# ViskaWei/VIT

Measured on AMD Instinct MI355X. Metric: images/sec ViT-B/16 224^2 bf16 train step, higher is better.
Workload: dtype bf16

## Files before the change

### include/vit_amd.h

```cpp
#ifndef VIT_AMD_H_
#define VIT_AMD_H_

#include <stddef.h>
#include <stdint.h>

#ifdef __cplusplus
extern "C" {
#endif

#define VIT_AMD_VERSION 100

typedef struct vit_ctx* vit_handle;
typedef void* vit_stream;

typedef enum { VIT_OK = 0, VIT_ERR_ARG = -1, VIT_ERR_HIP = -2, VIT_ERR_UNSUPPORTED = -3, VIT_ERR_WORKSPACE = -4 } vit_status;
typedef enum { VIT_F32 = 0, VIT_BF16 = 1 } vit_dtype;
typedef enum { VIT_ACT_NONE = 0, VIT_ACT_GELU = 1, VIT_ACT_DGELU = 2, VIT_ACT_GELU_GRAD = 3, VIT_ACT_MUL_AUX = 4 } vit_act;
typedef enum { VIT_LOSS_MSE = 0, VIT_LOSS_L1 = 1, VIT_LOSS_CE = 2, VIT_LOSS_SOFT_CE = 3, VIT_LOSS_BCE = 4 } vit_loss;

int vit_version(void);
const char* vit_last_error(void);

int vit_create(vit_handle* out, int device);
int vit_destroy(vit_handle h);
// ... 107 lines not shown
int vit_grad_sqnorm_acc(vit_handle h, const float* g, int64_t n, float* out, vit_stream stream);
int vit_adamw_step(vit_handle h, float* p, const float* g, float* m, float* v, void* p_bf16, int64_t n, float lr,
                   float beta1, float beta2, float eps, float weight_decay, int step, const float* sqnorm,
                   float max_norm, vit_stream stream);

#ifdef __cplusplus
}
#endif

#include "vit_amd_cov.h"
#include "vit_amd_optim.h"
#include "vit_amd_ema.h"
#include "vit_amd_droppath.h"
#include "vit_amd_layerscale.h"
#include "vit_amd_mix.h"

#endif
```

### vit_amd/_cabi.py

```python
from __future__ import annotations

import ctypes as C
import os
import re
import threading

_HERE = os.path.dirname(os.path.abspath(__file__))
LIB_PATH = os.environ.get("VIT_AMD_LIB") or os.path.join(_HERE, "lib", "libvit_amd.so")
HEADER_PATH = os.path.join(os.path.dirname(_HERE), "include", "vit_amd.h")

VIT_OK, VIT_ERR_WORKSPACE = 0, -4
VIT_F32, VIT_BF16 = 0, 1
ACT_NONE, ACT_GELU, ACT_DGELU, ACT_GELU_GRAD, ACT_MUL_AUX = 0, 1, 2, 3, 4
LOSS_MSE, LOSS_L1, LOSS_CE = 0, 1, 2
LOSS_SOFT_CE, LOSS_BCE = 3, 4
MIX_LABELS_F32, MIX_LABELS_I64 = 0, 1


class VitError(RuntimeError):
    pass


class GemmDesc(C.Structure):
    _fields_ = [
# ... 38 lines not shown

_P, _I, _F, _U64, _I64, _SZ = C.c_void_p, C.c_int, C.c_float, C.c_uint64, C.c_int64, C.c_size_t

_PROTOS = {
    "vit_version": [],
    "vit_last_error": [],
    "vit_create": [C.POINTER(_P), _I],
    "vit_destroy": [_P],
    "vit_set_workspace": [_P, _P, _SZ],
    "vit_workspace_needed": [],
    "vit_set_option": [C.c_char_p, _I],
    "vit_handle_set_option": [_P, C.c_char_p, _I],
    "vit_step_state_bind": [_P, _P],
    "vit_step_advance": [_P, _U64, _F, _F, _P],
    "vit_gemm": [_P, C.POINTER(GemmDesc), _P],
    "vit_last_gemm_kernel": [],
    "vit_linear_fwd": [_P, _P, _P, _P, _P, _I, _I, _I, _I, _I, _P, _F, _U64, _U64, _P, _P],
    "vit_linear_bwd_dx": [_P, _P, _P, _P, _I, _I, _I, _I, _P, _P],
    "vit_linear_bwd_dw": [_P, _P, _P, _P, _I, _I, _I, _I, _P],
    "vit_layernorm_fwd": [_P, _P, _P, _P, _P, _I, _P, _P, _I, _I, _F, _P],
    "vit_layernorm_fwd_residual": [_P, _P, _P, _I, _P, _P, _P, _P, _I, _P, _P, _I, _I, _F, _P],
    "vit_linear_bwd_dw_rows": [_P, _P, _I64, _P, _I64, _I, _P, _I, _I, _I, _I64, _I64, _P],
    "vit_colsum_rows": [_P, _P, _I, _I64, _P, _I, _I, _I64, _I64, _P],
    "vit_layernorm_fwd_residual_rows": [_P, _P, _I64, _P, _I, _P, _P, _P, _P, _I, _P, _P, _I, _I, _F, _P],
    "vit_layernorm_bwd_rows": [_P, _P, _I, _P, _P, _P, _P, _P, _I64, _P, _P, _P, _I, _I, _P, _I, _P, _F, _U64, _U64, _I64, _P],
    "vit_layernorm_bwd": [_P, _P, _I, _P, _P, _P, _P, _P, _P, _P, _P, _I, _I, _P],
    "vit_layernorm_bwd_fused": [_P, _P, _I, _P, _P, _P, _P, _P, _P, _P, _P, _I, _I, _P, _I, _P, _F, _U64, _U64, _P],
    "vit_attention_fwd": [_P, _P, _P, _P, _P, _I, _I, _I, _I, _I, _F, _F, _U64, _U64, _P],
    "vit_attention_bwd": [_P, _P, _P, _P, _P, _P, _P, _P, _I, _I, _I, _I, _I, _F, _F, _U64, _U64, _P, _P],
    "vit_attention_probs": [_P, _P, _P, _I, _I, _I, _I, _I, _F, _P],
# ... 156 lines not shown
```

### vit_amd/build.py

```python
from __future__ import annotations

import hashlib
import os
import subprocess
import sys
from concurrent.futures import ThreadPoolExecutor

HERE = os.path.dirname(os.path.abspath(__file__))
ROOT = os.path.dirname(HERE)
CSRC = os.path.join(HERE, "csrc")
OBJ = os.path.join(CSRC, "_build")
LIBDIR = os.path.join(HERE, "lib")
LIB = os.path.join(LIBDIR, "libvit_amd.so")
ARCH = "gfx950"
SOURCES = ["api.hip", "gemm.hip", "gemm2.hip", "layernorm.hip", "attention.hip", "attention_tiled.hip", "attention_resident.hip",
           "attention_pipe.hip", "attention_f32.hip", "elementwise.hip", "covariance.hip", "optim.hip", "ema.hip", "layerscale.hip", "mix.hip"]
HEADERS = [os.path.join(CSRC, "common.h"), os.path.join(CSRC, "attention.h"), os.path.join(ROOT, "include", "vit_amd.h"),
           os.path.join(ROOT, "include", "vit_amd_cov.h"), os.path.join(ROOT, "include", "vit_amd_optim.h"),
           os.path.join(ROOT, "include", "vit_amd_ema.h"), os.path.join(ROOT, "include", "vit_amd_droppath.h"),
           os.path.join(ROOT, "include", "vit_amd_layerscale.h"), os.path.join(ROOT, "include", "vit_amd_mix.h")]


def _hipcc() -> str:
    for c in (os.environ.get("HIPCC"), "/opt/rocm/bin/hipcc", "hipcc"):
        if c and (os.path.isabs(c) and os.path.exists(c) or not os.path.isabs(c)):
            return c
    raise RuntimeError("hipcc not found")


def _stamp(paths) -> str:
    h = hashlib.sha256()
    for p in paths:
        with open(p, "rb") as f:
            h.update(f.read())
    return h.hexdigest()
# ... 49 lines not shown
```

### vit_amd/csrc/api.hip

```cpp
#include <stdarg.h>
#include <stdio.h>
#include <string.h>

#include <algorithm>

#include "common.h"

struct vit_ctx {
  int device;
  void* ws;
  size_t ws_bytes;
  const void* step_state;
  int num_cus;
  int reserve_cus;
  int grad_accumulate;
  int lamb_passes;
};

namespace vit {

extern int g_gemm2_mode;
extern int g_attn_split, g_attn_bwd_fused;

static thread_local char g_err[512] = "";
thread_local char g_last_gemm[96] = "";

void set_error(const char* fmt, ...) {
  va_list ap;
  va_start(ap, fmt);
  vsnprintf(g_err, sizeof(g_err), fmt, ap);
  va_end(ap);
// ... 5 lines not shown
int ctx_num_cus(vit_handle h) {
  static int dflt = 0;
  if (h) return std::max(1, h->num_cus - (h->reserve_cus >= 0 ? h->reserve_cus : g_reserve_cus));
  if (!dflt) {
    int dev = 0, n = 0;
    if (hipGetDevice(&dev) == hipSuccess && hipDeviceGetAttribute(&n, hipDeviceAttributeMultiprocessorCount, dev) == hipSuccess && n > 0)
      dflt = n;
    else
      dflt = 256;
  }
  return std::max(1, dflt - g_reserve_cus);
}

int ctx_grad_accumulate(vit_handle h) { return h ? h->grad_accumulate : 0; }
int ctx_lamb_passes(vit_handle h) { return h ? h->lamb_passes : 7; }

static thread_local size_t g_ws_needed = 0;
void* ctx_claim(vit_handle h, size_t need_bytes, const char* who) {
  const size_t have = h ? h->ws_bytes : 0;
  if (h && h->ws && have >= need_bytes) return h->ws;
  g_ws_needed = need_bytes;
  set_error("%s: needs %zu workspace bytes, have %zu", who, need_bytes, have);
  return nullptr;
}

}

extern "C" {

int vit_version(void) { return VIT_AMD_VERSION; }
// ... 8 lines not shown
  VIT_HIP(hipGetDeviceCount(&n));
  VIT_CHECK(device >= 0 && device < n, VIT_ERR_ARG, "vit_create: device %d out of range (%d visible)", device, n);
  hipDeviceProp_t prop;
  VIT_HIP(hipGetDeviceProperties(&prop, device));
  VIT_CHECK(strncmp(prop.gcnArchName, "gfx950", 6) == 0, VIT_ERR_UNSUPPORTED,
            "vit_create: device %d is %s; this library is built for gfx950 (MI355X) only", device, prop.gcnArchName);
  vit_ctx* c = new vit_ctx();
  c->device = device;
  c->ws = nullptr;
  c->ws_bytes = 0;
  c->step_state = nullptr;
  c->num_cus = prop.multiProcessorCount > 0 ? prop.multiProcessorCount : 256;
  c->reserve_cus = -1;
  c->grad_accumulate = 0;
  c->lamb_passes = 7;
  *out = c;
  return VIT_OK;
}

int vit_destroy(vit_handle h) {
  delete h;
  return VIT_OK;
}

const char* vit_last_gemm_kernel(void) { return vit::g_last_gemm; }

int vit_set_option(const char* name, int value) {
  VIT_CHECK(name, VIT_ERR_ARG, "vit_set_option: null name");
  if (strcmp(name, "gemm_core") == 0) {
    VIT_CHECK(value == 0 || value == 1 || value == 5, VIT_ERR_ARG,
// ... 28 lines not shown
  if (strcmp(name, "reserve_cus") == 0) {
    VIT_CHECK(value >= -1 && value <= 128, VIT_ERR_ARG, "vit_handle_set_option: reserve_cus takes -1 (process default) or 0 .. 128");
    h->reserve_cus = value;
    return VIT_OK;
  }
  if (strcmp(name, "grad_accumulate") == 0) {
    VIT_CHECK(value == 0 || value == 1, VIT_ERR_ARG, "vit_handle_set_option: grad_accumulate takes 0 or 1");
    h->grad_accumulate = value;
    return VIT_OK;
  }
  if (strcmp(name, "lamb_passes") == 0) {
    VIT_CHECK(value >= 1 && value <= 7, VIT_ERR_ARG, "vit_handle_set_option: lamb_passes takes 1 .. 7 (bits: moments 1, ratios 2, apply 4)");
    h->lamb_passes = value;
    return VIT_OK;
  }
  vit::set_error("vit_handle_set_option: '%s' is not a per-handle option (reserve_cus, grad_accumulate, lamb_passes)", name);
  return VIT_ERR_ARG;
}

int vit_step_state_bind(vit_handle h, void* state) {
  VIT_CHECK(h, VIT_ERR_ARG, "vit_step_state_bind: null handle");
  VIT_CHECK(((uintptr_t)state & 15) == 0, VIT_ERR_ARG, "vit_step_state_bind: state must be 16-byte aligned");
  h->step_state = state;
  return VIT_OK;
}

int vit_set_workspace(vit_handle h, void* ws, size_t bytes) {
  VIT_CHECK(h, VIT_ERR_ARG, "vit_set_workspace: null handle");
  VIT_CHECK(((uintptr_t)ws & 255) == 0, VIT_ERR_ARG, "vit_set_workspace: workspace must be 256-byte aligned");
  h->ws = ws;
  h->ws_bytes = bytes;
// ... 5 lines not shown
```

### vit_amd/csrc/common.h

```cpp
#pragma once
#include <hip/hip_runtime.h>
#include <stdint.h>

#include "../../include/vit_amd.h"

namespace vit {

typedef __attribute__((ext_vector_type(8))) short bf16x8;
typedef __attribute__((ext_vector_type(4))) short bf16x4;
typedef __attribute__((ext_vector_type(4))) float f32x4;
typedef __attribute__((ext_vector_type(4))) int i32x4;
typedef __attribute__((ext_vector_type(2))) int i32x2;
typedef __attribute__((ext_vector_type(4))) unsigned u32x4;
typedef __attribute__((ext_vector_type(2))) unsigned u32x2;

#define LDS_AS __attribute__((address_space(3)))

void set_error(const char* fmt, ...);
extern thread_local char g_last_gemm[96];
#define VIT_CHECK(cond, code, ...)            \
  do {                                         \
    if (!(cond)) {                             \
      ::vit::set_error(__VA_ARGS__);           \
      return (code);                           \
// ... 256 lines not shown
  int accumulate;
  int grad_accumulate;
  int scratch;
  DropCfg drop;
  int drs;
  KRows kr;
  size_t slab_bytes, colsum_bytes, scratch_off, need;
  char* ws;
  char symbol[96];
};
int gemm_plan(vit_handle h, const vit_gemm_desc* d, KRows kr, GemmPlan* pl);
bool pp_plan(vit_handle h, const vit_gemm_desc* d, GemmPlan* pl);
int pp_launch(const GemmPlan& pl, const vit_gemm_desc* d, hipStream_t st);
int gemm_launch(vit_handle h, const vit_gemm_desc* d, hipStream_t st, int k_row_stride = 0, int k_rows = 0);

template <class Args>
static inline void fill_gemm_args(Args& a, const GemmPlan& pl, const vit_gemm_desc* d) {
  a.A = (const char*)d->A; a.B = (const char*)d->B; a.C = (char*)d->C;
  a.lda = d->lda; a.ldb = d->ldb; a.ldc = d->ldc;
  a.M = d->M; a.N = d->N; a.K = d->K;
  a.tiles_m = pl.tiles_m; a.tiles_n = pl.tiles_n;
  a.splits = pl.splits; a.k_per_split = pl.k_per_split;
  a.slab = pl.splits > 1 ? (float*)pl.ws : nullptr;
  a.bias = d->bias;
  a.aux_in = (const short*)d->aux_in; a.aux_out = (short*)d->aux_out; a.ldaux = d->ldaux;
  a.residual = d->residual; a.ldres = d->ldres;
  if (pl.accumulate && pl.splits == 1) { a.residual = (const float*)d->C; a.ldres = d->ldc; }
  a.alpha = d->alpha;
  a.act = d->act; a.c_dtype = d->c_dtype;
  a.drop = pl.drop;
// ... 6 lines not shown
```

### vit_amd/csrc/gemm.hip

```cpp
#include <algorithm>
#include <stdio.h>
#include <string.h>

#include "common.h"

namespace vit {

constexpr int BM = 128, BN = 128, BK = 64, NTHR = 256;
constexpr int STAGE_BYTES = (BM * BK + BN * BK) * 2;
constexpr int A_BYTES = BM * BK * 2;

struct GemmArgs {
  const char* A; const char* B; char* C;
  long lda, ldb, ldc;
  long a_bs, b_bs, c_bs;
  int M, N, K;
  int tiles_m, tiles_n;
  int splits, k_per_split;
  float* slab;
  const float* bias;
  const short* aux_in; short* aux_out; long ldaux;
  const float* residual; long ldres;
  float alpha;
  int act, c_dtype;
// ... 421 lines not shown
  for (long i = blockIdx.x * (long)blockDim.x + threadIdx.x; i < nvec; i += (long)gridDim.x * blockDim.x) {
    const long m = i / (N >> 2);
    const int n = (int)(i - m * (N >> 2)) << 2;
    float* c = C + m * ldc + n;
    *(f32x4*)c = *(const f32x4*)c + *(const f32x4*)(src + m * N + n);
  }
}

int launch_splitk_reduce(const float* slab, float* C, long ldc, int M, int N, int splits, float alpha, int accumulate,
                         hipStream_t st) {
  const long nvec = (long)M * (N / 4);
  const int blocks = (int)std::min<long>((nvec + 255) / 256, 2048);
  hipLaunchKernelGGL(splitk_reduce_kernel, dim3(blocks), dim3(256), 0, st, slab, C, ldc, M, N, splits, alpha, accumulate);
  VIT_LAUNCH_CHECK();
  return VIT_OK;
}

static bool al16(const void* p) { return ((uintptr_t)p & 15) == 0; }
static size_t round256(size_t bytes) { return (bytes + 255) & ~(size_t)255; }

static void split_plan(const vit_gemm_desc* d, int bk, int* splits_out, int* kps_out) {
  const int ktiles = cdiv(d->K, bk);
  int splits = d->split_k;
  if (splits < 0) {
    const int tiles = cdiv(d->M, BM) * cdiv(d->N, BN);
    splits = 1;
    if (tiles < 256) splits = std::min(std::max(1, 512 / tiles), std::max(1, ktiles / 4));
  }
  if (splits < 1) splits = 1;
  if (splits > ktiles) splits = ktiles;
// ... 141 lines not shown
  }
  rc = pl.core == GEMM_PP ? pp_launch(pl, d, st) : generic_launch(pl, d, st);
  if (rc == VIT_OK && pl.rope == PASS_BEHIND)
    rc = vit_rope_qk(h, d->C, d->c_dtype, d->rope_cos, d->rope_sin, d->M, d->rope_T, d->rope_cols / (2 * d->rope_dh), d->rope_dh,
                     d->ldc, 0, (vit_stream)st);
  if (rc == VIT_OK && pl.colsum == PASS_BEHIND)
    rc = vit_colsum(h, d->C, d->c_dtype, d->ldc, d->colsum_out, d->M, d->N, pl.grad_accumulate, (vit_stream)st);
  if (rc != VIT_OK || !pl.scratch) return rc;
  const long nvec = (long)d->M * (d->N / 4);
  hipLaunchKernelGGL(add_into_kernel, dim3((int)std::min<long>((nvec + 255) / 256, 2048)), dim3(256), 0, st, c_out, ldc_out,
                     (const float*)d->C, d->M, d->N);
  VIT_LAUNCH_CHECK();
  return VIT_OK;
}

}

extern "C" {

int vit_gemm(vit_handle h, const vit_gemm_desc* d, vit_stream stream) {
  return vit::gemm_launch(h, d, (hipStream_t)stream);
}

int vit_linear_fwd(vit_handle h, const void* x, const void* W, const float* bias, void* y, int y_dtype, int M, int N,
                   int K, int act, void* aux_out, float dropout_p, uint64_t seed, uint64_t site,
                   const float* residual, vit_stream stream) {
  vit_gemm_desc d = {};
  d.M = M; d.N = N; d.K = K; d.ab_dtype = VIT_BF16;
  d.A = x; d.lda = K; d.B = W; d.ldb = K; d.C = y; d.ldc = N; d.c_dtype = y_dtype;
  d.alpha = 1.f; d.bias = bias; d.act = act; d.aux_out = aux_out; d.ldaux = N;
  d.dropout_p = dropout_p; d.seed = seed; d.site = site; d.residual = residual; d.ldres = N;
  return vit::gemm_launch(h, &d, (hipStream_t)stream);
}

int vit_linear_bwd_dx(vit_handle h, const void* dy, const void* W, void* dx, int dx_dtype, int M, int N, int K,
                      const void* dgelu_aux_in, vit_stream stream) {
// ... 19 lines not shown
```

### vit_amd/csrc/gemm2.hip

```cpp
#include <algorithm>
#include <stdio.h>

#include "common.h"

namespace vit {

#define GLB_AS __attribute__((address_space(1)))

struct Gemm2Args {
  const char* A; const char* B; char* C;
  long lda, ldb, ldc;
  int M, N, K;
  int tiles_m, tiles_n, nblk;
  int splits, k_per_split;
  float* slab;
  const float* bias;
  const short* aux_in; short* aux_out; long ldaux;
  const float* residual; long ldres;
  float alpha;
  int act, c_dtype;
  DropCfg drop;
  int rpb, orb, roff;
  int drs;
  int lin_split;
// ... 261 lines not shown
      v += __shfl_xor(v, 8, 64);
      v += __shfl_xor(v, 16, 64);
      v += __shfl_xor(v, 32, 64);
      cs[r] = v;
    }
    if (lane < 8) {
      float* dst = p.colsum_part + (long)(m0 >> 7) * p.N + n;
      *(f32x4*)dst = (f32x4){cs[0], cs[1], cs[2], cs[3]};
      *(f32x4*)(dst + 4) = (f32x4){cs[4], cs[5], cs[6], cs[7]};
    }
  }
#undef EPI_STORE_C
#undef EPI_STORE_AUX
}

template <int A_T, int B_T, int EPI, int NSLOT>
__global__ __launch_bounds__(512, 2) void gemm3_kernel(Gemm2Args p) {
  resolve_drop(p.drop);
  constexpr int BM = 256, BN = 256, BK = 64;
  constexpr int HALF = 128 * BK * 2;
  static_assert(NSLOT == 8, "the ring arithmetic below is for 8 slots (two K-tiles of four half-tiles)");
  constexpr int DEPTH = NSLOT - 3, INFL = 2 * (DEPTH - 1);
  constexpr int SCR = 4096, CW = 64;
  constexpr int XA0 = 0, XB0 = 1, XB1 = 2, XA1 = 3;
  constexpr int RELAX = INFL + (((EPI >= 3 && EPI <= 6) || EPI == 8) ? 16 : 32);
  extern __shared__ __attribute__((aligned(16))) char smem[];

  const int tid = threadIdx.x, lane = tid & 63;
  const int wave = __builtin_amdgcn_readfirstlane(tid >> 6);
  const int wr = wave >> 2, wc = wave & 3, grp = wr;
  const int l15 = lane & 15, lg = lane >> 4;

  const int ntile = p.tiles_m * p.tiles_n;
  int split = blockIdx.y, bx = blockIdx.x;
  if (p.lin_split) {
    const int total = ntile * p.splits, lin = blockIdx.x;
    const int q = total >> 3, r = total & 7, xcd = lin & 7, within = lin >> 3;
    const int pos = (xcd < r ? xcd * (q + 1) : r * (q + 1) + (xcd - r) * q) + within;
    split = pos / ntile;
    bx = pos - split * ntile;
  }
  const int k_begin = split * p.k_per_split;
  const int k_end = min(p.K, k_begin + p.k_per_split);
  const int nk = (k_end - k_begin) / BK;
  const int nblk = p.nblk;
  const int my_tiles = (ntile - bx + nblk - 1) / nblk;
  const int T = my_tiles * nk;

  int offA[2], offB[2];
#pragma unroll
// ... 205 lines not shown
        PP_KTILE2
      } else {
        PP_KTILE4
      }
      relaxed = 0;
      a1 = a2;
      bb1 = bb2;
      cursor_next(a2, bb2);
      kb ^= 4 * HALF;
    }
    {
      int tm, tn;
      tile_coords(jt, tm, tn);
      if (grp == 0) __builtin_amdgcn_s_barrier();
      char* scr = smem + 8 * HALF + wave * SCR;
      if constexpr (EPI >= 3) pp_epilogue<EPI, 8>(acc, scr, p, tm * BM + wr * 128, tn * BN + wc * 64, split, lane);
      else tile_epilogue<8, 4, CW, EPI>(acc, scr, p, tm * BM + wr * 128, tn * BN + wc * 64, split, lane);
      if (grp == 1) __builtin_amdgcn_s_barrier();
      relaxed = 1;
    }
  }
  if (grp == 0) __builtin_amdgcn_s_barrier();
#undef PP_READ_A
#undef PP_READ_B
#undef PP_MFMA
#undef PP_STAGE
#undef PP_KTILE2
#undef PP_KTILE4
#undef PP_LOADED
#undef PP_MFMA2
  asm volatile("s_waitcnt vmcnt(0)" ::: "memory");
}

template <int AT, int BT, int EPI>
static int launch_stag(const Gemm2Args& a, dim3 grid, hipStream_t st) {
  constexpr int smem = 160 * 1024;
  static bool attr_done = false;
  auto fn = gemm3_kernel<AT, BT, EPI, 8>;
  if (!attr_done) {
    VIT_HIP(hipFuncSetAttribute((const void*)fn, hipFuncAttributeMaxDynamicSharedMemorySize, smem));
    attr_done = true;
  }
  hipLaunchKernelGGL(fn, grid, dim3(512), smem, st, a);
  VIT_LAUNCH_CHECK();
  return VIT_OK;
}
// ... 105 lines not shown
  return true;
}

int pp_launch(const GemmPlan& pl, const vit_gemm_desc* d, hipStream_t st) {
  Gemm2Args a;
  fill_gemm_args(a, pl, d);
  a.nblk = pl.nblk; a.lin_split = pl.lin_split; a.grp2 = pl.grp2;
  a.colsum_part = pl.colsum == PASS_FUSED ? (float*)pl.ws : nullptr;
  a.rope_cos = d->rope_cos; a.rope_sin = d->rope_sin; a.rope_T = d->rope_T; a.rope_dh = d->rope_dh; a.rope_cols = d->rope_cols;
  int r = launch_stag_cfg(a, pl.a_t, pl.b_t, pl.epi, pl.grid, st);
  if (r == VIT_OK && a.colsum_part)
    r = launch_reduce_partials(a.colsum_part, a.tiles_m * 2, d->N, d->colsum_out, d->N, d->colsum_out, pl.grad_accumulate, st);
  if (r == VIT_OK && pl.splits > 1)
    r = launch_splitk_reduce(a.slab, (float*)d->C, (long)d->ldc, d->M, d->N, pl.splits, d->alpha, pl.accumulate, st);
  return r;
}


__global__ __launch_bounds__(256) void dw_rows_kernel(const short* __restrict__ dy, long ldy, const short* __restrict__ x,
                                                      long ldx, float* __restrict__ dW, long ldw, int B, int s, int kps,
                                                      int splits, int accumulate) {
  constexpr int R = 128;
  __shared__ __attribute__((aligned(16))) short ys[R][64];
  __shared__ __attribute__((aligned(16))) short xs[R][64];
  const int t = threadIdx.x, lane = t & 63, wave = t >> 6, l15 = lane & 15, lg = lane >> 4;
  const int wn = (wave >> 1) * 32, wk = (wave & 1) * 32;
  const int n0 = blockIdx.x * 64, k0 = blockIdx.y * 64;
  f32x4 acc[2][2], tot[2][2];
#pragma unroll
  for (int i = 0; i < 2; ++i)
// ... 146 lines not shown
```

### vit_amd/engine.py

```python
from __future__ import annotations

import collections
import gc
import math
import os
from typing import Callable, Dict, List, Optional, Tuple

import torch

from . import _cabi
from . import functional as vf
from ._cabi import ACT_GELU, LOSS_BCE, LOSS_CE, LOSS_L1, LOSS_MSE, LOSS_SOFT_CE, VitError
from .config import ViTConfig

ALIGN = 8

EMBED = "vit.embeddings."
PROJ = EMBED + "patch_embeddings.projection"
LayerNames = collections.namedtuple("LayerNames", "ln1 q wo ln2 fc1 fc2")
_LAYER_STEMS = LayerNames("layernorm_before", "attention.attention.query", "attention.output.dense", "layernorm_after",
                          "intermediate.dense", "output.dense")
LAMBDA = "lambda1"
_SCALED = (("layer_scale1", "attention.output.dense"), ("layer_scale2", "output.dense"))
ScaledLinear = collections.namedtuple("ScaledLinear", "Wf bf dW_raw db_raw")
# ... 167 lines not shown
        self._arena_key = None
        self._arenas: Dict[bool, Arena] = {}
        self.act: Dict[str, object] = {}
        self.tmp: Dict[str, torch.Tensor] = {}
        self._Mp = 0
        self._rows: Optional[Tuple[Rows, Rows]] = None
        self._rope, self._rope_key = None, None
        self.precision = "f32"
        self.base_seed = int(torch.initial_seed()) & 0x7FFFFFFFFFFFFFFF
        self.step_counter = 0
        self._last = None
        self.side_stream: Optional[torch.cuda.Stream] = None
        self._side_handle = None
        self._main_handle = None
        self.reserve_cus = -1
        self._side_reads: Dict[int, object] = {}
        self._on_side = _SideHop(self)
        self.overlap_dw = "auto"
        self.cls_tail = os.environ.get("VIT_CLS_TAIL", "1") != "0"
        self._accum = False
        self._gen = 0
        self.grad_ready_cb: Optional[Callable[[int, int], None]] = None
        self.version_fn: Callable[[], int] = lambda: self.flat._version

    def set_soft_loss(self, name: str) -> int:
        if self.loss_kind != LOSS_CE:
            raise ValueError("soft-target losses belong to classification (task_type 'cls')")
        kinds = {"ce": LOSS_SOFT_CE, "bce": LOSS_BCE}
        if name not in kinds:
            raise ValueError(f"soft_loss must be one of {sorted(kinds)}, got {name!r}")
# ... 109 lines not shown
        if self._ls is None or self._fold_epoch != self._shadow_epoch:
            self.fold_layer_scale()

    def handle(self):
        if self._main_handle is None or self._main_handle.device_index != self._device_index():
            self._main_handle = self._new_handle()
        return self._main_handle

    def _device_index(self) -> int:
        dev = self.flat.device
        return dev.index if dev.index is not None else torch.cuda.current_device()

    def _new_handle(self):
        h = _cabi.Handle(self._device_index())
        h.set_option("reserve_cus", self.reserve_cus)
        if self._accum:
            h.set_option("grad_accumulate", 1)
        return h

    def set_reserve_cus(self, n: int):
        self.reserve_cus = int(n)
        for h in (self._main_handle, self._side_handle):
            if h is not None:
                h.set_option("reserve_cus", self.reserve_cus)

    def mark_shadow_fresh(self):
        self._shadow_version = self.version_fn()

    def w16(self, name: str) -> torch.Tensor:
        return self.layout.view(self.shadow if self.precision == "bf16" else self.flat, name)

    def g(self, name: str) -> torch.Tensor:
        return self.layout.view(self.grads, name)

    def _scaled(self, stem: str) -> Optional[ScaledLinear]:
        return None if self._ls is None else self._ls.views.get(stem)

    def W(self, stem: str) -> torch.Tensor:
        v = self._scaled(stem)
# ... 233 lines not shown
            if raw:
                vf._h(out).set_option("grad_accumulate", 0)
            try:
                if r.stride > 1:
                    return vf.linear_bwd_dw_rows(dy, x, out, row_stride=r.stride, full_rows=r.Mp, ldx=ldx)
                vf.gemm(dy, x, M=N, N=K, K=r.n, a_trans=True, b_trans=True, ldb=ldx, out=out, split_k=-1)
            finally:
                if raw:
                    vf._h(out).set_option("grad_accumulate", 1)
            if side is not None:
                ev = torch.cuda.Event()
                ev.record(side)
                self._side_reads[dy.data_ptr()] = ev
        return out

    def _unfold_layer_scale(self, i: int):
        if self._ls is not None:
            with self._on_side:
                vf.layer_scale_grad(self._ls.table, self._accum, first=2 * i, count=2)

    def _before_write(self, buf):
        if self.side_stream is None:
            return
        ev = self._side_reads.pop(buf.data_ptr(), None)
        if ev is not None:
            torch.cuda.current_stream(self.flat.device).wait_event(ev)

    def _join_side(self):
        if self.side_stream is not None:
            torch.cuda.current_stream(self.flat.device).wait_stream(self.side_stream)
# ... 30 lines not shown
    def _ln_bwd(self, r: Rows, name: str, dy, x, mean, rstd, dres, dx, dyn=None, dbias=None, dropout=vf.NO_DROP,
                dres_row_stride: int = 0, path=None):
        vf.layernorm_bwd_rows(dy, x, self.p(name + ".weight"), mean, rstd, dres, dx, self.dW(name), self.db(name), dyn=dyn,
                              dbias=dbias, dropout=dropout, dres_row_stride=dres_row_stride, row_stride=r.stride, full_rows=r.M,
                              path=path)

    def _fc2_dy(self, r: Rows, i: int, ph: float, seed: int, pd=None) -> dict:
        if i < 0:
            return {}
        return dict(dyn=r.dy, dbias=self.db(self.names[i].fc2), dropout=(ph, seed, self._site(i, 2)), path=self._path(pd, i, 1))

    def _tail_bwd(self, r: Rows, i: int, dx, dx_out, ph: float, seed: int, pd=None):
        c, a, nm = self.cfg, self.act, self.names[i]
        D, Fd, n = c.hidden_size, c.intermediate_size, r.n
        strided = r.stride > 1
        self._dw(r, r.dy, r.g[i], self.dW(nm.fc2))
        self._before_write(r.dU)
        vf.gemm(r.dy, self.W(nm.fc2), M=n, N=Fd, K=D, b_trans=True, out=r.dU, act=vf.ACT_MUL_AUX, aux_in=r.u[i],
                colsum_out=None if strided else self.db(nm.fc1))
        if strided:
            vf.colsum_rows(r.dU, self.db(nm.fc1), row_stride=r.stride, full_rows=r.Mp)
        self._dw(r, r.dU, r.h2[i], self.dW(nm.fc1))
        vf.gemm(r.dU, self.W(nm.fc1), M=n, N=D, K=Fd, b_trans=True, out=r.dh)
        self._before_write(r.dy2)
        self._ln_bwd(r, nm.ln2, r.dh, r.x1[i], r.mean2[i], r.rstd2[i], dx, dx_out, dyn=r.dy2, dbias=self.db(nm.wo),
                     dropout=(ph, seed, self._site(i, 1)), path=self._path(pd, i, 0))
        self._dw(r, r.dy2, a["ctx"][i], self.dW(nm.wo), ldx=r.stride * D)
        vf.gemm(r.dy2, self.W(nm.wo), M=n, N=D, K=D, b_trans=True, out=r.dctx, ldc=r.stride * D)

    def _set_accumulate(self, on: bool):
        for h in (self._main_handle, self._side_handle):
            if h is not None:
                h.set_option("grad_accumulate", int(on))

    def backward(self, dloss: torch.Tensor, need_dx: bool = False, gen: Optional[int] = None, accumulate: bool = False):
        with vf.use_handle(self.handle()):
            if not accumulate:
                return self._backward(dloss, need_dx, gen)
            self._accum = True
            try:
                self._set_accumulate(True)
                return self._backward(dloss, need_dx, gen)
# ... 24 lines not shown
        self._setup_side()
        dx, spare = r.dx
        self._ln_bwd(r, "vit.layernorm", r.dlast.view(-1, D), r.xL, r.meanF, r.rstdF, None, dx,
                     **self._fc2_dy(r, L - 1, ph, seed, pd))
        self._notify(self.layout.tail_start, self.layout.n_trainable)
        for i in reversed(range(L)):
            self._tail_bwd(r, i, dx, spare, ph, seed, pd)
            dx, spare = spare, dx
            self._before_write(t["dqkv"])
            vf.attention_bwd(a["qkv"][i], a["ctx"][i], r.dctx, a["lse"][i], B, H, T, dh, scale,
                             dropout=(pa, seed, self._site(i, 0)), dqkv=t["dqkv"], delta=t["delta"],
                             colsum_out=None if rope is not None else self._qkv_bias(i, self.grads), ctx_lo=a["ctx_lo"][i])
            if rope is not None:
                vf.rope_qk(t["dqkv"], rope[0], rope[1], T, H, dh, inverse=True)
                vf.colsum(t["dqkv"], out=self._qkv_bias(i, self.grads), accumulate=self._accum)
            self._dw(full, t["dqkv"], a["h1"][i], self._qkv_w(i, self.grads))
            vf.gemm(t["dqkv"], self._qkv16(i), M=full.n, N=D, K=3 * D, b_trans=True, out=t["dh"])
            self._before_write(t["dy"])
            dres, rejoin = dx, 0
            if r is not full:
                rejoin, r = r.stride, full
                dx, spare = full.dx
            self._ln_bwd(full, self.names[i].ln1, t["dh"], a["x"][i].view(M, D), a["mean1"][i], a["rstd1"][i], dres, spare,
                         dres_row_stride=rejoin, **self._fc2_dy(full, i - 1, ph, seed, pd))
            dx, spare = spare, dx
            self._unfold_layer_scale(i)
            self._notify(*self.layout.layer_ranges[i])
        dpos = self.g(EMBED + "position_embeddings").view(T, D) if c.pos_encoding_type == "learned" else None
        vf.embed_finish_bwd(dx.view(B, T, D), self.g(EMBED + "cls_token").view(D), dpos, dropout=(ph, seed, 0),
                            dpatch=t["dpatch"])
        vf.colsum(t["dpatch"], out=self.db(PROJ), accumulate=self._accum)
# ... 9 lines not shown
```

### vit_amd/functional.py

```python
from __future__ import annotations

import ctypes as C
from typing import Optional, Tuple

import torch

from . import _cabi
from ._cabi import ACT_DGELU, ACT_GELU, ACT_GELU_GRAD, ACT_MUL_AUX, ACT_NONE, LOSS_BCE, LOSS_CE, LOSS_L1, LOSS_MSE, LOSS_SOFT_CE, VIT_BF16, VIT_F32, GemmDesc

_DT = {torch.float32: VIT_F32, torch.bfloat16: VIT_BF16}


def _stream(t: torch.Tensor) -> int:
    return torch.cuda.current_stream(t.device).cuda_stream


_HANDLE_OVERRIDE: Optional[_cabi.Handle] = None


def _h(t: torch.Tensor) -> _cabi.Handle:
    if not t.is_cuda:
        raise _cabi.VitError("vit_amd kernels need tensors on an MI355X (cuda/hip device); there is no CPU path")
    return _HANDLE_OVERRIDE if _HANDLE_OVERRIDE is not None else _cabi.handle_for(t.device)

# ... 63 lines not shown
        _chk(colsum_out, torch.float32, "gemm colsum_out")
        if colsum_out.numel() != N:
            raise _cabi.VitError(f"gemm: colsum_out must have N={N} elements")
        d.colsum_out = colsum_out.data_ptr()
    if rope is not None:
        cos, sin, rT, rdh, rcols = rope
        _chk(cos, torch.float32, "gemm rope cos")
        _chk(sin, torch.float32, "gemm rope sin")
        if cos.numel() != rT * (rdh // 2) or sin.numel() != cos.numel():
            raise _cabi.VitError(f"gemm: rope tables must be [T={rT}, head_dim/2={rdh // 2}]")
        d.rope_cos, d.rope_sin, d.rope_T, d.rope_dh, d.rope_cols = cos.data_ptr(), sin.data_ptr(), int(rT), int(rdh), int(rcols)
    h.call("vit_gemm", C.byref(d), _stream(a))
    return out


def linear_fwd(x, W, bias=None, *, out_dtype=torch.bfloat16, act=ACT_NONE, aux_out=None, dropout: Dropout = NO_DROP,
               residual=None, out=None):
    M, K = x.shape
    N = W.shape[0]
    return gemm(x, W, M=M, N=N, K=K, out=out, out_dtype=out_dtype, bias=bias, act=act, aux_out=aux_out, dropout=dropout,
                residual=residual)


def linear_bwd_dx(dy, W, *, out_dtype=torch.bfloat16, dgelu_aux=None, out=None):
    M, N = dy.shape
    K = W.shape[1]
    return gemm(dy, W, M=M, N=K, K=N, b_trans=True, out=out, out_dtype=out_dtype,
                act=ACT_DGELU if dgelu_aux is not None else ACT_NONE, aux_in=dgelu_aux)


# ... 627 lines not shown
```

Measured before the change: 7942.

## Group attention-out and QKV weight-gradient GEMMs into one split-K launch

Adds a grouped split-K GEMM path that runs the Wo and QKV weight-gradient GEMMs for a layer in a single persistent launch, with one grouped reduction kernel afterwards. Each of these GEMMs alone has fewer tiles than there are CUs, so putting their tiles together is meant to fill the machine better and cut launch and reduce overhead. In exchange, the Wo dW now waits until the QKV dW is ready, which delays it, and the split-K slab for both outputs needs more workspace.

Result: no change. 7954, median of 3 (+0.2%).

```diff
diff --git a/include/vit_amd.h b/include/vit_amd.h
--- a/include/vit_amd.h
+++ b/include/vit_amd.h
@@ -145,5 +145,6 @@
 #include "vit_amd_droppath.h"
 #include "vit_amd_layerscale.h"
 #include "vit_amd_mix.h"
+#include "vit_amd_group.h"
 
 #endif
diff --git a/include/vit_amd_group.h b/include/vit_amd_group.h
--- /dev/null
+++ b/include/vit_amd_group.h
@@ -0,0 +1,14 @@
+#ifndef VIT_AMD_GROUP_H_
+#define VIT_AMD_GROUP_H_
+
+#ifdef __cplusplus
+extern "C" {
+#endif
+
+int vit_gemm_group(vit_handle h, const vit_gemm_desc* descs, int n, vit_stream stream);
+
+#ifdef __cplusplus
+}
+#endif
+
+#endif
diff --git a/vit_amd/_cabi.py b/vit_amd/_cabi.py
--- a/vit_amd/_cabi.py
+++ b/vit_amd/_cabi.py
@@ -76,6 +76,7 @@
     "vit_step_state_bind": [_P, _P],
     "vit_step_advance": [_P, _U64, _F, _F, _P],
     "vit_gemm": [_P, C.POINTER(GemmDesc), _P],
+    "vit_gemm_group": [_P, C.POINTER(GemmDesc), _I, _P],
     "vit_last_gemm_kernel": [],
     "vit_linear_fwd": [_P, _P, _P, _P, _P, _I, _I, _I, _I, _I, _P, _F, _U64, _U64, _P, _P],
     "vit_linear_bwd_dx": [_P, _P, _P, _P, _I, _I, _I, _I, _P, _P],
diff --git a/vit_amd/build.py b/vit_amd/build.py
--- a/vit_amd/build.py
+++ b/vit_amd/build.py
@@ -18,7 +18,8 @@
 HEADERS = [os.path.join(CSRC, "common.h"), os.path.join(CSRC, "attention.h"), os.path.join(ROOT, "include", "vit_amd.h"),
            os.path.join(ROOT, "include", "vit_amd_cov.h"), os.path.join(ROOT, "include", "vit_amd_optim.h"),
            os.path.join(ROOT, "include", "vit_amd_ema.h"), os.path.join(ROOT, "include", "vit_amd_droppath.h"),
-           os.path.join(ROOT, "include", "vit_amd_layerscale.h"), os.path.join(ROOT, "include", "vit_amd_mix.h")]
+           os.path.join(ROOT, "include", "vit_amd_layerscale.h"), os.path.join(ROOT, "include", "vit_amd_mix.h"),
+           os.path.join(ROOT, "include", "vit_amd_group.h")]
 
 
 def _hipcc() -> str:
diff --git a/vit_amd/csrc/api.hip b/vit_amd/csrc/api.hip
--- a/vit_amd/csrc/api.hip
+++ b/vit_amd/csrc/api.hip
@@ -15,6 +15,7 @@
   int reserve_cus;
   int grad_accumulate;
   int lamb_passes;
+  int gemm_group;
 };
 
 namespace vit {
@@ -50,6 +51,7 @@
 
 int ctx_grad_accumulate(vit_handle h) { return h ? h->grad_accumulate : 0; }
 int ctx_lamb_passes(vit_handle h) { return h ? h->lamb_passes : 7; }
+int ctx_gemm_group(vit_handle h) { return h ? h->gemm_group : 1; }
 
 static thread_local size_t g_ws_needed = 0;
 void* ctx_claim(vit_handle h, size_t need_bytes, const char* who) {
@@ -88,6 +90,7 @@
   c->reserve_cus = -1;
   c->grad_accumulate = 0;
   c->lamb_passes = 7;
+  c->gemm_group = 1;
   *out = c;
   return VIT_OK;
 }
@@ -146,7 +149,12 @@
     h->lamb_passes = value;
     return VIT_OK;
   }
-  vit::set_error("vit_handle_set_option: '%s' is not a per-handle option (reserve_cus, grad_accumulate, lamb_passes)", name);
+  if (strcmp(name, "gemm_group") == 0) {
+    VIT_CHECK(value == 0 || value == 1, VIT_ERR_ARG, "vit_handle_set_option: gemm_group takes 0 or 1");
+    h->gemm_group = value;
+    return VIT_OK;
+  }
+  vit::set_error("vit_handle_set_option: '%s' is not a per-handle option (reserve_cus, grad_accumulate, lamb_passes, gemm_group)", name);
   return VIT_ERR_ARG;
 }
 
diff --git a/vit_amd/csrc/common.h b/vit_amd/csrc/common.h
--- a/vit_amd/csrc/common.h
+++ b/vit_amd/csrc/common.h
@@ -294,6 +294,21 @@
 int pp_launch(const GemmPlan& pl, const vit_gemm_desc* d, hipStream_t st);
 int gemm_launch(vit_handle h, const vit_gemm_desc* d, hipStream_t st, int k_row_stride = 0, int k_rows = 0);
 
+struct GemmGroupPlan {
+  int n, ntile;
+  int splits, k_per_split;
+  int tiles_m[4], tiles_n[4];
+  int cum[3];
+  int accumulate[4];
+  long slab_off[4], slice_stride;
+  size_t need;
+  char* ws;
+  char symbol[96];
+};
+bool pp_group_plan(vit_handle h, const vit_gemm_desc* descs, int n, GemmGroupPlan* gp);
+int pp_group_launch(const GemmGroupPlan& gp, const vit_gemm_desc* descs, hipStream_t st);
+int ctx_gemm_group(vit_handle h);
+
 template <class Args>
 static inline void fill_gemm_args(Args& a, const GemmPlan& pl, const vit_gemm_desc* d) {
   a.A = (const char*)d->A; a.B = (const char*)d->B; a.C = (char*)d->C;
diff --git a/vit_amd/csrc/gemm.hip b/vit_amd/csrc/gemm.hip
--- a/vit_amd/csrc/gemm.hip
+++ b/vit_amd/csrc/gemm.hip
@@ -459,6 +459,27 @@
   hipLaunchKernelGGL(splitk_reduce_kernel, dim3(blocks), dim3(256), 0, st, slab, C, ldc, M, N, splits, alpha, accumulate);
   VIT_LAUNCH_CHECK();
   return VIT_OK;
+}
+
+struct GroupReduceMember { float* C; long ldc, slab_off, vec_end; int nq, accumulate; };
+struct GroupReduceArgs { const float* slab; long slice_stride; int splits; GroupReduceMember m[4]; };
+__global__ void splitk_reduce_group_kernel(GroupReduceArgs a) {
+  const long nvec = a.m[3].vec_end;
+  for (long i = blockIdx.x * (long)blockDim.x + threadIdx.x; i < nvec; i += (long)gridDim.x * blockDim.x) {
+    const bool s1 = i >= a.m[0].vec_end, s2 = i >= a.m[1].vec_end, s3 = i >= a.m[2].vec_end;
+#define GRP_SEL(F) (s3 ? a.m[3].F : s2 ? a.m[2].F : s1 ? a.m[1].F : a.m[0].F)
+    const long j = i - (s3 ? a.m[2].vec_end : s2 ? a.m[1].vec_end : s1 ? a.m[0].vec_end : 0);
+    const int nq = GRP_SEL(nq);
+    const long m = j / nq;
+    const int n = (int)(j - m * nq) << 2;
+    const float* s = a.slab + GRP_SEL(slab_off) + m * (nq << 2) + n;
+    f32x4 v = *(const f32x4*)s;
+    for (int k = 1; k < a.splits; ++k) v += *(const f32x4*)(s + k * a.slice_stride);
+    float* c = GRP_SEL(C) + m * GRP_SEL(ldc) + n;
+    if (GRP_SEL(accumulate)) v += *(const f32x4*)c;
+#undef GRP_SEL
+    *(f32x4*)c = v;
+  }
 }
 
 static bool al16(const void* p) { return ((uintptr_t)p & 15) == 0; }
@@ -630,12 +651,56 @@
   return VIT_OK;
 }
 
+int gemm_group_launch(vit_handle h, const vit_gemm_desc* descs, int n, hipStream_t st) {
+  VIT_CHECK(descs && n >= 1 && n <= 4, VIT_ERR_ARG, "vit_gemm_group: takes 1 .. 4 descriptors (n=%d)", n);
+  size_t need = 0;
+  for (int i = 0; i < n; ++i) {
+    GemmPlan pl;
+    const int rc = gemm_plan(h, &descs[i], KRows{0, 0}, &pl);
+    if (rc != VIT_OK) return rc;
+    need = std::max(need, pl.need);
+    memcpy(g_last_gemm, pl.symbol, sizeof(g_last_gemm));
+  }
+  GemmGroupPlan gp;
+  if (!pp_group_plan(h, descs, n, &gp)) {
+    if (need && !ctx_claim(h, need, "vit_gemm_group")) return VIT_ERR_WORKSPACE;
+    for (int i = 0; i < n; ++i) {
+      const int rc = gemm_launch(h, &descs[i], st);
+      if (rc != VIT_OK) return rc;
+    }
+    return VIT_OK;
+  }
+  memcpy(g_last_gemm, gp.symbol, sizeof(g_last_gemm));
+  if (!(gp.ws = (char*)ctx_claim(h, gp.need, "vit_gemm_group"))) return VIT_ERR_WORKSPACE;
+  const int rc = pp_group_launch(gp, descs, st);
+  if (rc != VIT_OK) return rc;
+  GroupReduceArgs a = {};
+  a.slab = (const float*)gp.ws; a.slice_stride = gp.slice_stride; a.splits = gp.splits;
+  long vec = 0;
+  for (int i = 0; i < 4; ++i) {
+    if (i < gp.n) {
+      const vit_gemm_desc* d = &descs[i];
+      vec += (long)d->M * (d->N / 4);
+      a.m[i] = GroupReduceMember{(float*)d->C, (long)d->ldc, gp.slab_off[i], vec, d->N / 4, gp.accumulate[i]};
+    } else {
+      a.m[i] = a.m[gp.n - 1];
+    }
+  }
+  hipLaunchKernelGGL(splitk_reduce_group_kernel, dim3((int)std::min<long>((vec + 255) / 256, 2048)), dim3(256), 0, st, a);
+  VIT_LAUNCH_CHECK();
+  return VIT_OK;
+}
+
 }
 
 extern "C" {
 
 int vit_gemm(vit_handle h, const vit_gemm_desc* d, vit_stream stream) {
   return vit::gemm_launch(h, d, (hipStream_t)stream);
+}
+
+int vit_gemm_group(vit_handle h, const vit_gemm_desc* descs, int n, vit_stream stream) {
+  return vit::gemm_group_launch(h, descs, n, (hipStream_t)stream);
 }
 
 int vit_linear_fwd(vit_handle h, const void* x, const void* W, const float* bias, void* y, int y_dtype, int M, int N,
diff --git a/vit_amd/csrc/gemm2.hip b/vit_amd/csrc/gemm2.hip
--- a/vit_amd/csrc/gemm2.hip
+++ b/vit_amd/csrc/gemm2.hip
@@ -1,4 +1,5 @@
 #include <algorithm>
+#include <limits.h>
 #include <stdio.h>
 
 #include "common.h"
@@ -299,8 +300,8 @@
 #undef EPI_STORE_AUX
 }
 
-template <int A_T, int B_T, int EPI, int NSLOT>
-__global__ __launch_bounds__(512, 2) void gemm3_kernel(Gemm2Args p) {
+template <int A_T, int B_T, int EPI, int NSLOT, int GROUP>
+__device__ __forceinline__ void gemm3_body(Gemm2Args p, int g_split, int g_bx) {
   resolve_drop(p.drop);
   constexpr int BM = 256, BN = 256, BK = 64;
   constexpr int HALF = 128 * BK * 2;
@@ -317,8 +318,8 @@
   const int l15 = lane & 15, lg = lane >> 4;
 
   const int ntile = p.tiles_m * p.tiles_n;
-  int split = blockIdx.y, bx = blockIdx.x;
-  if (p.lin_split) {
+  int split = GROUP ? g_split : blockIdx.y, bx = GROUP ? g_bx : blockIdx.x;
+  if (!GROUP && p.lin_split) {
     const int total = ntile * p.splits, lin = blockIdx.x;
     const int q = total >> 3, r = total & 7, xcd = lin & 7, within = lin >> 3;
     const int pos = (xcd < r ? xcd * (q + 1) : r * (q + 1) + (xcd - r) * q) + within;
@@ -554,7 +555,7 @@
       tile_coords(jt, tm, tn);
       if (grp == 0) __builtin_amdgcn_s_barrier();
       char* scr = smem + 8 * HALF + wave * SCR;
-      if constexpr (EPI >= 3) pp_epilogue<EPI, 8>(acc, scr, p, tm * BM + wr * 128, tn * BN + wc * 64, split, lane);
+      if constexpr (EPI >= 3) pp_epilogue<EPI, 8>(acc, scr, p, tm * BM + wr * 128, tn * BN + wc * 64, GROUP ? 0 : split, lane);
       else tile_epilogue<8, 4, CW, EPI>(acc, scr, p, tm * BM + wr * 128, tn * BN + wc * 64, split, lane);
       if (grp == 1) __builtin_amdgcn_s_barrier();
       relaxed = 1;
@@ -570,6 +571,45 @@
 #undef PP_LOADED
 #undef PP_MFMA2
   asm volatile("s_waitcnt vmcnt(0)" ::: "memory");
+}
+
+template <int A_T, int B_T, int EPI, int NSLOT>
+__global__ __launch_bounds__(512, 2) void gemm3_kernel(Gemm2Args p) {
+  gemm3_body<A_T, B_T, EPI, NSLOT, 0>(p, 0, 0);
+}
+
+struct Gemm2GroupMember {
+  const char* A; const char* B;
+  long lda, ldb, slab_off;
+  int M, N, tiles_m, tiles_n;
+};
+struct Gemm2GroupArgs {
+  Gemm2Args base;
+  Gemm2GroupMember m[4];
+  int cum[3];
+  int ntile;
+  long slice_stride;
+};
+
+template <int A_T, int B_T, int EPI, int NSLOT>
+__global__ __launch_bounds__(512, 2) void gemm3_group_kernel(Gemm2GroupArgs g) {
+  const int total = g.ntile * g.base.splits, lin = blockIdx.x;
+  const int q = total >> 3, r = total & 7, xcd = lin & 7, within = lin >> 3;
+  const int pos = (xcd < r ? xcd * (q + 1) : r * (q + 1) + (xcd - r) * q) + within;
+  const int split = pos / g.ntile;
+  const int ft = pos - split * g.ntile;
+  const bool s1 = ft >= g.cum[0], s2 = ft >= g.cum[1], s3 = ft >= g.cum[2];
+#define GRP_SEL(F) (s3 ? g.m[3].F : s2 ? g.m[2].F : s1 ? g.m[1].F : g.m[0].F)
+  Gemm2Args p = g.base;
+  p.A = GRP_SEL(A); p.B = GRP_SEL(B);
+  p.lda = GRP_SEL(lda); p.ldb = GRP_SEL(ldb);
+  p.M = GRP_SEL(M); p.N = GRP_SEL(N);
+  p.tiles_m = GRP_SEL(tiles_m); p.tiles_n = GRP_SEL(tiles_n);
+  p.nblk = p.tiles_m * p.tiles_n;
+  p.slab = g.base.slab + (long)split * g.slice_stride + GRP_SEL(slab_off);
+#undef GRP_SEL
+  const int first = s3 ? g.cum[2] : s2 ? g.cum[1] : s1 ? g.cum[0] : 0;
+  gemm3_body<A_T, B_T, EPI, NSLOT, 1>(p, split, ft - first);
 }
 
 template <int AT, int BT, int EPI>
@@ -705,6 +745,65 @@
   if (r == VIT_OK && pl.splits > 1)
     r = launch_splitk_reduce(a.slab, (float*)d->C, (long)d->ldc, d->M, d->N, pl.splits, d->alpha, pl.accumulate, st);
   return r;
+}
+
+bool pp_group_plan(vit_handle h, const vit_gemm_desc* descs, int n, GemmGroupPlan* gp) {
+  if (n < 2 || n > 4 || !ctx_gemm_group(h)) return false;
+  const int accum = ctx_grad_accumulate(h);
+  long ntile = 0, floats = 0;
+  for (int i = 0; i < n; ++i) {
+    const vit_gemm_desc* d = &descs[i];
+    if (d->ab_dtype != VIT_BF16 || !d->a_trans || !d->b_trans || d->c_dtype != VIT_F32) return false;
+    if (d->bias || d->act != VIT_ACT_NONE || d->dropout_p != 0.f || d->residual || d->rows_per_batch != 0 || d->colsum_out ||
+        d->rope_cos || d->alpha != 1.0f || d->aux_in || d->aux_out || d->split_k >= 0)
+      return false;
+    if (d->K != descs[0].K || !pp_shape_ok(d->M, d->N, d->K, d->lda, d->ldb)) return false;
+    gp->tiles_m[i] = d->M / 256; gp->tiles_n[i] = d->N / 256;
+    gp->slab_off[i] = floats;
+    if (i > 0) gp->cum[i - 1] = (int)ntile;
+    ntile += (long)gp->tiles_m[i] * gp->tiles_n[i];
+    floats += (long)d->M * d->N;
+    gp->accumulate[i] = d->accumulate || accum;
+  }
+  for (int i = n; i < 4; ++i) gp->cum[i - 1] = INT_MAX;
+  const int slots = ctx_num_cus(h);
+  if (ntile >= slots) return false;
+  int splits, kps;
+  pp_split_plan(slots, (int)ntile, descs[0].K, -1, &splits, &kps);
+  if (splits < 2) return false;
+  gp->n = n; gp->ntile = (int)ntile;
+  gp->splits = splits; gp->k_per_split = kps;
+  gp->slice_stride = floats;
+  gp->need = (size_t)splits * floats * sizeof(float);
+  snprintf(gp->symbol, sizeof(gp->symbol), "gemm3_group_kernel<1, 1, 7, 8>");
+  return true;
+}
+
+int pp_group_launch(const GemmGroupPlan& gp, const vit_gemm_desc* descs, hipStream_t st) {
+  constexpr int smem = 160 * 1024;
+  Gemm2GroupArgs g = {};
+  g.base.K = descs[0].K;
+  g.base.splits = gp.splits; g.base.k_per_split = gp.k_per_split;
+  g.base.slab = (float*)gp.ws;
+  g.base.alpha = 1.f; g.base.c_dtype = VIT_F32; g.base.drs = 1; g.base.lin_split = 1;
+  for (int i = 0; i < 4; ++i) {
+    const int j = std::min(i, gp.n - 1);
+    const vit_gemm_desc* d = &descs[j];
+    g.m[i] = Gemm2GroupMember{(const char*)d->A, (const char*)d->B, (long)d->lda, (long)d->ldb, gp.slab_off[j],
+                              d->M, d->N, gp.tiles_m[j], gp.tiles_n[j]};
+  }
+  for (int i = 0; i < 3; ++i) g.cum[i] = gp.cum[i];
+  g.ntile = gp.ntile;
+  g.slice_stride = gp.slice_stride;
+  static bool attr_done = false;
+  auto fn = gemm3_group_kernel<1, 1, 7, 8>;
+  if (!attr_done) {
+    VIT_HIP(hipFuncSetAttribute((const void*)fn, hipFuncAttributeMaxDynamicSharedMemorySize, smem));
+    attr_done = true;
+  }
+  hipLaunchKernelGGL(fn, dim3(gp.ntile * gp.splits), dim3(512), smem, st, g);
+  VIT_LAUNCH_CHECK();
+  return VIT_OK;
 }
 
 
diff --git a/vit_amd/engine.py b/vit_amd/engine.py
--- a/vit_amd/engine.py
+++ b/vit_amd/engine.py
@@ -205,6 +205,7 @@
         self._side_handle = None
         self._main_handle = None
         self.reserve_cus = -1
+        self.gemm_group = True
         self._side_reads: Dict[int, object] = {}
         self._on_side = _SideHop(self)
         self.overlap_dw = "auto"
@@ -344,6 +345,7 @@
     def _new_handle(self):
         h = _cabi.Handle(self._device_index())
         h.set_option("reserve_cus", self.reserve_cus)
+        h.set_option("gemm_group", int(self.gemm_group))
         if self._accum:
             h.set_option("grad_accumulate", 1)
         return h
@@ -353,6 +355,12 @@
         for h in (self._main_handle, self._side_handle):
             if h is not None:
                 h.set_option("reserve_cus", self.reserve_cus)
+
+    def set_gemm_group(self, on: bool):
+        self.gemm_group = bool(on)
+        for h in (self._main_handle, self._side_handle):
+            if h is not None:
+                h.set_option("gemm_group", int(self.gemm_group))
 
     def mark_shadow_fresh(self):
         self._shadow_version = self.version_fn()
@@ -616,6 +624,24 @@
                 self._side_reads[dy.data_ptr()] = ev
         return out
 
+    def _dw_group(self, r: Rows, members):
+        raws = [self._accum and self._ls is not None and m[2].data_ptr() in self._ls.raw_ptrs for m in members]
+        with self._on_side as side:
+            h = vf._h(members[0][2])
+            if any(raws):
+                h.set_option("grad_accumulate", 0)
+            try:
+                vf.gemm_group([(dy, x, out, ldx, self._accum and not raw) for (dy, x, out, ldx), raw in zip(members, raws)],
+                              K=r.n)
+            finally:
+                if any(raws):
+                    h.set_option("grad_accumulate", 1)
+            if side is not None:
+                ev = torch.cuda.Event()
+                ev.record(side)
+                for m in members:
+                    self._side_reads[m[0].data_ptr()] = ev
+
     def _unfold_layer_scale(self, i: int):
         if self._ls is not None:
             with self._on_side:
@@ -676,6 +702,7 @@
         c, a, nm = self.cfg, self.act, self.names[i]
         D, Fd, n = c.hidden_size, c.intermediate_size, r.n
         strided = r.stride > 1
+        grouped = i < c.num_hidden_layers - 1
         self._dw(r, r.dy, r.g[i], self.dW(nm.fc2))
         self._before_write(r.dU)
         vf.gemm(r.dy, self.W(nm.fc2), M=n, N=Fd, K=D, b_trans=True, out=r.dU, act=vf.ACT_MUL_AUX, aux_in=r.u[i],
@@ -687,7 +714,8 @@
         self._before_write(r.dy2)
         self._ln_bwd(r, nm.ln2, r.dh, r.x1[i], r.mean2[i], r.rstd2[i], dx, dx_out, dyn=r.dy2, dbias=self.db(nm.wo),
                      dropout=(ph, seed, self._site(i, 1)), path=self._path(pd, i, 0))
-        self._dw(r, r.dy2, a["ctx"][i], self.dW(nm.wo), ldx=r.stride * D)
+        if not grouped:
+            self._dw(r, r.dy2, a["ctx"][i], self.dW(nm.wo), ldx=r.stride * D)
         vf.gemm(r.dy2, self.W(nm.wo), M=n, N=D, K=D, b_trans=True, out=r.dctx, ldc=r.stride * D)
 
     def _set_accumulate(self, on: bool):
@@ -742,7 +770,11 @@
             if rope is not None:
                 vf.rope_qk(t["dqkv"], rope[0], rope[1], T, H, dh, inverse=True)
                 vf.colsum(t["dqkv"], out=self._qkv_bias(i, self.grads), accumulate=self._accum)
-            self._dw(full, t["dqkv"], a["h1"][i], self._qkv_w(i, self.grads))
+            if i < L - 1:
+                self._dw_group(full, [(full.dy2, a["ctx"][i], self.dW(self.names[i].wo), D),
+                                      (t["dqkv"], a["h1"][i], self._qkv_w(i, self.grads), None)])
+            else:
+                self._dw(full, t["dqkv"], a["h1"][i], self._qkv_w(i, self.grads))
             vf.gemm(t["dqkv"], self._qkv16(i), M=full.n, N=D, K=3 * D, b_trans=True, out=t["dh"])
             self._before_write(t["dy"])
             dres, rejoin = dx, 0
diff --git a/vit_amd/functional.py b/vit_amd/functional.py
--- a/vit_amd/functional.py
+++ b/vit_amd/functional.py
@@ -101,6 +101,26 @@
     return out
 
 
+def gemm_group(members, *, K: int):
+    descs = (GemmDesc * len(members))()
+    for d, (dy, x, out, ldx, accumulate) in zip(descs, members):
+        if dy.dtype != x.dtype or dy.dtype not in _DT:
+            raise _cabi.VitError(f"gemm_group: operands must both be bf16 or both f32 (got {dy.dtype}, {x.dtype})")
+        _chk(out, torch.float32, "gemm_group out")
+        M, N = out.shape
+        d.M, d.N, d.K = M, N, K
+        d.a_trans, d.b_trans = 1, 1
+        d.ab_dtype = _DT[dy.dtype]
+        d.A, d.lda = dy.data_ptr(), M
+        d.B, d.ldb = x.data_ptr(), ldx if ldx is not None else N
+        d.C, d.ldc, d.c_dtype = out.data_ptr(), N, VIT_F32
+        d.alpha = 1.0
+        d.ldaux = d.ldres = N
+        d.split_k = -1
+        d.accumulate = int(accumulate)
+    _h(members[0][0]).call("vit_gemm_group", descs, len(members), _stream(members[0][0]))
+
+
 def linear_fwd(x, W, bias=None, *, out_dtype=torch.bfloat16, act=ACT_NONE, aux_out=None, dropout: Dropout = NO_DROP,
                residual=None, out=None):
     M, K = x.shape
```
